# donydchen/matchnerf

Measured on AMD Instinct MI355X. Metric: rendered rays/sec (3-view, 64 samples/ray), higher is better.
Workload: dtype f32; 1 GPU

## Files before the change

matchnerf_amd/csrc/decoder.hip:

```cpp
#include "decoder_staged.hpp"

#define PP_STAGES 12
#define PP_PHASES 28
struct PPSched {
  int seg_first[PP_STAGES];
  int n_seg[PP_STAGES];
};

template <int SP>
struct SmemPP {
  static constexpr int TEAM = 128, TILE = 256;
  static constexpr int RING_FLOATS = 4 * SEG_CAP_FLOATS;
  static constexpr int TAIL_F = ((TAIL_FLOATS + 255) / 256) * 256;
  static constexpr int HDR_FLOATS = PP_STAGES * 256;
  static constexpr int RS_FLOATS = TILE * 4;
  static constexpr int TOTAL_FLOATS = RING_FLOATS + TAIL_F + HDR_FLOATS + RS_FLOATS + 64;
  static_assert(TEAM * 64 <= SEG_CAP_FLOATS, "a team's attention scratch must fit one ring slot");
  static_assert(TOTAL_FLOATS * 4 <= 160 * 1024, "LDS budget of one CU");
};
__device__ __host__ constexpr int pp_p0(int s, int fs = 2) {
  if (s == 0) return 1 + 8 * fs;
  constexpr int t[PP_STAGES] = {17, 33, 33, 33, 33, 33, 32, 33, 17, 33, 17, 9};
  return t[s];
}
__device__ __host__ constexpr int pp_stream_pieces(int k, int fs = 2) {
  if (k == 0) return 1 + 8 * fs;
  constexpr int t[20] = {17, 33, 33, 32, 33, 32, 33, 32, 33, 32, 33, 32, 32, 17, 33, 32, 17, 20, 9, 11};
  return t[k];
}
__device__ __host__ constexpr int pp_stream_off_floats(int k, int fs = 2) {
  int o = 0;
  for (int m = 0; m < k; ++m) o += pp_stream_pieces(m, fs) * 256;
  return o;
}
__device__ __host__ constexpr int pp_seg_first(int s) {
  constexpr int t[PP_STAGES] = {0, 1, 2, 4, 6, 8, 11, 10, 13, 14, 16, 18};
  return t[s];
}
__device__ __host__ constexpr int pp_seg_off_floats(int s, int i, int fs = 2) { return pp_stream_off_floats(pp_seg_first(s) + i, fs); }
constexpr int PP_DMA_IN_M = 0;
static_assert(PP_DMA_IN_M == 0, "requests inside matrix phases take single pieces 2 tw + half + 8 k");
__device__ __host__ constexpr int pp_km(int n) {
  const int enc_stage = 7;
  if (n < 3 || n > 11 || n == enc_stage + 1) return 0;
  const int fit = pp_p0(n) / 8;
  return fit < PP_DMA_IN_M ? fit : PP_DMA_IN_M;
}
__device__ __host__ constexpr int pp_p1(int s) {
  constexpr int t[PP_STAGES] = {0, 0, 32, 32, 32, 32, 32, 0, 0, 32, 20, 0};
  return t[s];
}


template <int CTRL, int ROW_MASK = 0xF>
__device__ __forceinline__ float dpp_get0(float v) {
  return __int_as_float(__builtin_amdgcn_update_dpp(0, __float_as_int(v), CTRL, ROW_MASK, 0xF, true));
}
__device__ __forceinline__ float readlane_f(float v, int l) {
  return __int_as_float(__builtin_amdgcn_readlane(__float_as_int(v), l));
}
__device__ __forceinline__ float wave_sum_dpp(float v) {
  v = dpp_group_sum<16>(v);
  return (readlane_f(v, 0) + readlane_f(v, 16)) + (readlane_f(v, 32) + readlane_f(v, 48));
}
__device__ __forceinline__ float wave_exclusive_sum_dpp(float v, int lane) {
  float x = dpp_get0<0x111>(v);
  const float c15 = readlane_f(v, 15), c31 = readlane_f(v, 31), c47 = readlane_f(v, 47);
  x = lane == 16 ? c15 : (lane == 32 ? c31 : (lane == 48 ? c47 : x));
  x += dpp_get0<0x111>(x);
  x += dpp_get0<0x112>(x);
  x += dpp_get0<0x114>(x);
  x += dpp_get0<0x118>(x);
  const float t0 = readlane_f(x, 15), t1 = readlane_f(x, 31), t2 = readlane_f(x, 47);
  const float t01 = t0 + t1;
  return x + (lane >= 48 ? t01 + t2 : (lane >= 32 ? t01 : (lane >= 16 ? t0 : 0.0f)));
}

template <int SP, bool PADDED>
__device__ __forceinline__ void ray_attention_pp(const float* q_lds, const float* k_lds, const float* vt_lds, float* o_lds,
                                                 int a_ray, int a_hp, int s_q, int lane, int S) {
  constexpr int G = SP / 4;
  constexpr int NH = SP >= 128 ? 1 : 2;
#pragma unroll 1
  for (int h0 = 0; h0 < 2; h0 += NH) {
    f32x4 sc[NH][G];
    float4 q4[NH];
    const float* kb[NH];
    const float* vb[NH];
#pragma unroll
    for (int hh = 0; hh < NH; ++hh) {
      const int head = 2 * a_hp + h0 + hh;
      q4[hh] = *reinterpret_cast<const float4*>(q_lds + s_q * 16 + head * 4);
      kb[hh] = k_lds + ((a_ray * 4 + head) * SP + (lane & 3)) * 4;
      vb[hh] = vt_lds + ((a_ray * 4 + head) * 4 + (lane & 3)) * SP;
    }
#pragma unroll
    for (int g = 0; g < G; g += 2) {
      float4 ka[NH], kc[NH];
      f32x4 ta[NH], tc[NH];
#pragma unroll
      for (int hh = 0; hh < NH; ++hh) {
        ka[hh] = *reinterpret_cast<const float4*>(kb[hh] + g * 16);
        kc[hh] = *reinterpret_cast<const float4*>(kb[hh] + g * 16 + 16);
      }
#pragma unroll
      for (int hh = 0; hh < NH; ++hh) {
        ta[hh] = mfma4(ka[hh].x, q4[hh].x, (f32x4){0.f, 0.f, 0.f, 0.f});
        tc[hh] = mfma4(kc[hh].x, q4[hh].x, (f32x4){0.f, 0.f, 0.f, 0.f});
      }
#pragma unroll
      for (int hh = 0; hh < NH; ++hh) {
        ta[hh] = mfma4(ka[hh].y, q4[hh].y, ta[hh]);
        tc[hh] = mfma4(kc[hh].y, q4[hh].y, tc[hh]);
      }
#pragma unroll
      for (int hh = 0; hh < NH; ++hh) {
        ta[hh] = mfma4(ka[hh].z, q4[hh].z, ta[hh]);
        tc[hh] = mfma4(kc[hh].z, q4[hh].z, tc[hh]);
      }
#pragma unroll
      for (int hh = 0; hh < NH; ++hh) {
        sc[hh][g] = mfma4(ka[hh].w, q4[hh].w, ta[hh]);
        sc[hh][g + 1] = mfma4(kc[hh].w, q4[hh].w, tc[hh]);
      }
    }
    float mx[NH];
#pragma unroll
    for (int hh = 0; hh < NH; ++hh) {
      float mx4[4] = {-3.0e38f, -3.0e38f, -3.0e38f, -3.0e38f};
      if constexpr (!PADDED) {
#pragma unroll
        for (int g = 0; g < G; ++g)
#pragma unroll
          for (int r = 0; r < 4; ++r) mx4[r] = fmaxf(mx4[r], sc[hh][g][r]);
      } else {
        int s_keys = S;
        asm volatile("" : "+s"(s_keys));
#pragma unroll
        for (int g = 0; g < G; ++g)
#pragma unroll
          for (int r = 0; r < 4; ++r) {
            const float v = (4 * g + r < s_keys) ? sc[hh][g][r] : -3.0e38f;
            sc[hh][g][r] = v;
            mx4[r] = fmaxf(mx4[r], v);
          }
      }
      mx[hh] = fmaxf(fmaxf(mx4[0], mx4[1]), fmaxf(mx4[2], mx4[3]));
    }
    float ls4[NH][4];
    f32x4 oa[NH], ob[NH];
#pragma unroll
    for (int hh = 0; hh < NH; ++hh) {
#pragma unroll
      for (int r = 0; r < 4; ++r) ls4[hh][r] = 0.f;
      oa[hh] = (f32x4){0.f, 0.f, 0.f, 0.f};
      ob[hh] = (f32x4){0.f, 0.f, 0.f, 0.f};
    }
#pragma unroll
    for (int g = 0; g < G; g += 2) {
      float4 va[NH], vc[NH];
#pragma unroll
      for (int hh = 0; hh < NH; ++hh) {
        va[hh] = *reinterpret_cast<const float4*>(vb[hh] + 4 * g);
        vc[hh] = *reinterpret_cast<const float4*>(vb[hh] + 4 * g + 4);
      }
#pragma unroll
      for (int u = 0; u < 2; ++u)
#pragma unroll
        for (int hh = 0; hh < NH; ++hh)
#pragma unroll
          for (int r = 0; r < 4; ++r) {
            const float pr = __builtin_amdgcn_exp2f(sc[hh][g + u][r] - mx[hh]);
            sc[hh][g + u][r] = pr;
            ls4[hh][r] += pr;
          }
#pragma unroll
      for (int hh = 0; hh < NH; ++hh) {
        oa[hh] = mfma4(va[hh].x, sc[hh][g][0], oa[hh]);
        ob[hh] = mfma4(vc[hh].x, sc[hh][g + 1][0], ob[hh]);
      }
#pragma unroll
      for (int hh = 0; hh < NH; ++hh) {
        oa[hh] = mfma4(va[hh].y, sc[hh][g][1], oa[hh]);
        ob[hh] = mfma4(vc[hh].y, sc[hh][g + 1][1], ob[hh]);
      }
#pragma unroll
      for (int hh = 0; hh < NH; ++hh) {
        oa[hh] = mfma4(va[hh].z, sc[hh][g][2], oa[hh]);
        ob[hh] = mfma4(vc[hh].z, sc[hh][g + 1][2], ob[hh]);
      }
#pragma unroll
      for (int hh = 0; hh < NH; ++hh) {
        oa[hh] = mfma4(va[hh].w, sc[hh][g][3], oa[hh]);
        ob[hh] = mfma4(vc[hh].w, sc[hh][g + 1][3], ob[hh]);
      }
    }
#pragma unroll
    for (int hh = 0; hh < NH; ++hh) {
      const int head = 2 * a_hp + h0 + hh;
      const float lsum = (ls4[hh][0] + ls4[hh][1]) + (ls4[hh][2] + ls4[hh][3]);
      const float il = 1.0f / lsum;
      *reinterpret_cast<float4*>(o_lds + s_q * 16 + head * 4) =
          make_float4((oa[hh][0] + ob[hh][0]) * il, (oa[hh][1] + ob[hh][1]) * il, (oa[hh][2] + ob[hh][2]) * il,
                      (oa[hh][3] + ob[hh][3]) * il);
    }
  }
}

template <bool PADDED, class Wait>
__device__ __forceinline__ void ray_attention_pp256(const float* q_lds, const float* k0, const float* vt0, const float* k1,
                                                    const float* vt1, float* o_lds, int a_hp, int s_q, int lane, int S, int first,
                                                    Wait wait_other) {
  constexpr int HS = 128, G = HS / 4;
  float m0 = -3.0e38f, m1 = -3.0e38f, l0 = 0.f, l1 = 0.f;
  f32x4 o0 = {0.f, 0.f, 0.f, 0.f}, o1 = {0.f, 0.f, 0.f, 0.f};
#pragma unroll 1
  for (int it = 0; it < 4; ++it) {
    if (it == 2) wait_other();
    const int half = it < 2 ? first : 1 - first;
    const int hsel = it & 1;
    const int head = 2 * a_hp + hsel;
    const float* kh = half == 0 ? k0 : k1;
    const float* vh = half == 0 ? vt0 : vt1;
    int n_keys = S - half * HS;
    n_keys = n_keys < 0 ? 0 : (n_keys > HS ? HS : n_keys);
    const float m_run = hsel ? m1 : m0, l_run = hsel ? l1 : l0;
    const float4 q4 = *reinterpret_cast<const float4*>(q_lds + s_q * 16 + head * 4);
    const float* kb = kh + (head * HS + (lane & 3)) * 4;
    const float* vb = vh + (head * 4 + (lane & 3)) * HS;
    f32x4 sc[G];
#pragma unroll
    for (int g = 0; g < G; g += 2) {
      const float4 ka = *reinterpret_cast<const float4*>(kb + g * 16);
      const float4 kc = *reinterpret_cast<const float4*>(kb + g * 16 + 16);
      f32x4 ta = mfma4(ka.x, q4.x, (f32x4){0.f, 0.f, 0.f, 0.f});
      f32x4 tc = mfma4(kc.x, q4.x, (f32x4){0.f, 0.f, 0.f, 0.f});
      ta = mfma4(ka.y, q4.y, ta);
      tc = mfma4(kc.y, q4.y, tc);
      ta = mfma4(ka.z, q4.z, ta);
      tc = mfma4(kc.z, q4.z, tc);
      sc[g] = mfma4(ka.w, q4.w, ta);
      sc[g + 1] = mfma4(kc.w, q4.w, tc);
    }
    float mx4[4] = {-3.0e38f, -3.0e38f, -3.0e38f, -3.0e38f};
    if constexpr (!PADDED) {
#pragma unroll
      for (int g = 0; g < G; ++g)
#pragma unroll
        for (int r = 0; r < 4; ++r) mx4[r] = fmaxf(mx4[r], sc[g][r]);
    } else {
      int s_keys = __builtin_amdgcn_readfirstlane(n_keys);
      asm volatile("" : "+s"(s_keys));
#pragma unroll
      for (int g = 0; g < G; ++g)
#pragma unroll
        for (int r = 0; r < 4; ++r) {
          const float v = (4 * g + r < s_keys) ? sc[g][r] : -3.0e38f;
          sc[g][r] = v;
          mx4[r] = fmaxf(mx4[r], v);
        }
    }
    const float m_new = fmaxf(m_run, fmaxf(fmaxf(mx4[0], mx4[1]), fmaxf(mx4[2], mx4[3])));
    float ls4[4] = {0.f, 0.f, 0.f, 0.f};
    f32x4 oa = {0.f, 0.f, 0.f, 0.f}, ob = {0.f, 0.f, 0.f, 0.f};
#pragma unroll
    for (int g = 0; g < G; g += 2) {
      const float4 va = *reinterpret_cast<const float4*>(vb + 4 * g);
      const float4 vc = *reinterpret_cast<const float4*>(vb + 4 * g + 4);
#pragma unroll
      for (int u = 0; u < 2; ++u)
#pragma unroll
        for (int r = 0; r < 4; ++r) {
          const float pr = __builtin_amdgcn_exp2f(sc[g + u][r] - m_new);
          sc[g + u][r] = pr;
          ls4[r] += pr;
        }
      oa = mfma4(va.x, sc[g][0], oa);
      ob = mfma4(vc.x, sc[g + 1][0], ob);
      oa = mfma4(va.y, sc[g][1], oa);
      ob = mfma4(vc.y, sc[g + 1][1], ob);
      oa = mfma4(va.z, sc[g][2], oa);
      ob = mfma4(vc.z, sc[g + 1][2], ob);
      oa = mfma4(va.w, sc[g][3], oa);
      ob = mfma4(vc.w, sc[g + 1][3], ob);
    }
    const float f_old = __builtin_amdgcn_exp2f(m_run - m_new);
    const float l_new = l_run * f_old + ((ls4[0] + ls4[1]) + (ls4[2] + ls4[3]));
    f32x4 o_new;
#pragma unroll
    for (int d = 0; d < 4; ++d) o_new[d] = (hsel ? o1[d] : o0[d]) * f_old + (oa[d] + ob[d]);
    if (hsel) {
      m1 = m_new, l1 = l_new, o1 = o_new;
    } else {
      m0 = m_new, l0 = l_new, o0 = o_new;
    }
  }
  {
    const float i0 = 1.0f / l0, i1 = 1.0f / l1;
    *reinterpret_cast<float4*>(o_lds + s_q * 16 + (2 * a_hp) * 4) = make_float4(o0[0] * i0, o0[1] * i0, o0[2] * i0, o0[3] * i0);
    *reinterpret_cast<float4*>(o_lds + s_q * 16 + (2 * a_hp + 1) * 4) = make_float4(o1[0] * i1, o1[1] * i1, o1[2] * i1, o1[3] * i1);
  }
}

template <int SP, int FS = 2, bool POSES = false, int NPK = 3>
__global__ __launch_bounds__(512, 2) void decoder_pp_kernel(
    mnerf_decoder D, DecSched sch, PPSched pps, mnerf_view view0, mnerf_rays Rl, const float* __restrict__ cond,
    float* __restrict__ out_rgb, float* __restrict__ out_depth, float* __restrict__ out_opacity,
    float* __restrict__ dbg_rgb_s, float* __restrict__ dbg_sigma, const float* __restrict__ ext_ndc,
    const float* __restrict__ ext_dir) {
  constexpr int Sp = SP;
  using SM = SmemPP<SP>;
  constexpr int TEAM = SM::TEAM;
  extern __shared__ __attribute__((aligned(16))) float smem[];
  const unsigned ring_lds = __builtin_amdgcn_groupstaticsize();
  const unsigned tail_lds = ring_lds + SM::RING_FLOATS * 4u;
  const unsigned hdr_lds = tail_lds + SM::TAIL_F * 4u;
  float* tail = smem + SM::RING_FLOATS;
  float* rs_all = tail + SM::TAIL_F + SM::HDR_FLOATS;
  float* ln_lds = rs_all + SM::RS_FLOATS;

  const int tid = threadIdx.x;
  const int lane0 = tid & 63;
  const int wave = __builtin_amdgcn_readfirstlane(tid >> 6);
  const int team = wave >> 2, tw = wave & 3;
  const mnerf_rays& R = Rl;
  const int S = R.n_samples;
  constexpr bool WIDE = SP == 256;
  static_assert(!WIDE || (!POSES && FS == 2), "the 256-sample instance exists for the shipped shape without a pose table");
  const int rays_per_team = WIDE ? 0 : TEAM / Sp, rays_per_tile = WIDE ? 1 : 2 * rays_per_team;
  const int n_tiles = (R.n_rays + rays_per_tile - 1) / rays_per_tile;
  const int CS = D.cond_stride;
  const float freq_mul = R.legacy_coord ? 1.0f : 3.14159265358979323846f;
  const float wm1 = (float)(R.width - 1), hm1 = (float)(R.height - 1);
  float* rs_lds = rs_all + team * TEAM * 4;
  float* att = smem + (team == 0 ? 3 : 2) * SEG_CAP_FLOATS;
  float* k_lds = att;
  float* vt_lds = att + TEAM * 16;
  float* q_lds = att + TEAM * 32;
  float* o_lds = att + TEAM * 48;
  const float* k_other = smem + (team == 0 ? 2 : 3) * SEG_CAP_FLOATS;
  const float* vt_other = k_other + TEAM * 16;
  float* rows_lds = smem + 1 * SEG_CAP_FLOATS + team * 4096;
  const unsigned rows_lds_addr = ring_lds + (unsigned)(1 * SEG_CAP_FLOATS + team * 4096) * 4u;

#define PP_SLOT_LDS(s_, i_) (ring_lds + (unsigned)(2 * ((s_)&1) + (i_)) * (SEG_CAP_FLOATS * 4u))
#define PP_HDR_LDS(s_) (hdr_lds + (unsigned)(s_) * 1024u)
#define PP_SEG_SRC(s_, i_) (D.wstream + pp_seg_off_floats(s_, i_, FS))

  if (tid < SMALL_FIXED) ln_lds[tid] = D.small_[tid];
  if (tid < 2) reinterpret_cast<unsigned*>(ln_lds)[48 + tid] = 0u;
  const unsigned team_ctr_lds = hdr_lds + (unsigned)(SM::HDR_FLOATS + SM::RS_FLOATS + 48 + team) * 4u;
  int team_epoch = 0;
  const unsigned other_ctr_lds = hdr_lds + (unsigned)(SM::HDR_FLOATS + SM::RS_FLOATS + 48 + (1 - team)) * 4u;
  int tile_it = 0;
  auto wait_other_team = [&](int arrivals) {
    const int want = 4 * arrivals;
    for (;;) {
      unsigned v;
      asm volatile("ds_read_b32 %0, %1\n\ts_waitcnt lgkmcnt(0)" : "=v"(v) : "v"(other_ctr_lds) : "memory");
      if ((int)((unsigned)__builtin_amdgcn_readfirstlane((int)v) - (unsigned)want) >= 0) break;
      __builtin_amdgcn_s_sleep(1);
    }
  };
  {
    const unsigned voff = (unsigned)lane0 * 16u;
    for (int p = wave; p < pp_stream_pieces(19); p += 8)
      glds16_s(D.wstream + pp_stream_off_floats(19, FS) + p * 256, voff, __builtin_amdgcn_readfirstlane(tail_lds + (unsigned)p * 1024u));
    for (int s = wave; s < PP_STAGES; s += 8) glds16_s(PP_SEG_SRC(s, 0), voff, __builtin_amdgcn_readfirstlane(PP_HDR_LDS(s)));
    for (int p = wave; p < pp_p0(0, FS); p += 8)
      glds16_s(PP_SEG_SRC(0, 0) + p * 256, voff, __builtin_amdgcn_readfirstlane(PP_SLOT_LDS(0, 0) + (unsigned)p * 1024u));
  }
  segment_wait();
  __syncthreads();
  if (team == 1) __syncthreads();

  int tile_begin = blockIdx.x, tile_end = n_tiles, tile_step = gridDim.x;
  if (gridDim.x >= 8) {
    const int xcd = blockIdx.x & 7;
    tile_begin = (int)((long long)n_tiles * xcd / 8) + (int)(blockIdx.x >> 3);
    tile_end = (int)((long long)n_tiles * (xcd + 1) / 8);
    tile_step = ((int)gridDim.x - xcd + 7) >> 3;
  }
#ifdef MNERF_TIMELINE
  int pp_tl_tile = -1, pp_ph = 0;
#define PP_STAMPED(sync_)                                                                                      \
  do {                                                                                                         \
    unsigned long long* o_ = (sch.tl && lane0 == 0 && blockIdx.x < 32 && pp_tl_tile >= 0 && pp_tl_tile < 4)     \
                                 ? sch.tl + ((((size_t)blockIdx.x * 4 + pp_tl_tile) * 8 + wave) * PP_PHASES + pp_ph) * 2 \
                                 : nullptr;                                                                    \
    __builtin_amdgcn_sched_barrier(0);                                                                         \
    if (o_) o_[0] = __builtin_amdgcn_s_memtime();                                                              \
    sync_;                                                                                                     \
    if (o_) o_[1] = __builtin_amdgcn_s_memtime();                                                              \
    __builtin_amdgcn_sched_barrier(0);                                                                         \
    ++pp_ph;                                                                                                   \
  } while (0)
#else
#define PP_STAMPED(sync_)                    \
  do {                                       \
    __builtin_amdgcn_sched_barrier(0);       \
    sync_;                                   \
    __builtin_amdgcn_sched_barrier(0);       \
  } while (0)
#endif
#define PP_SYNC() PP_STAMPED(__syncthreads())
#define PP_TSYNC() PP_STAMPED(wave_group_sync(team_ctr_lds, 4, team_epoch, (int)hw_lane()))
#define PP_NOSYNC() PP_STAMPED((void)0)
  auto stage_dma = [&](int s, int half) {
    const unsigned voff = hw_lane() * 16u;
    int twl = tw;
    asm volatile("" : "+s"(twl));
    for (int i = 0; i < 2; ++i) {
      const int pieces = i == 0 ? pp_p0(s, FS) : pp_p1(s);
      const unsigned base = PP_SLOT_LDS(s, i);
      const int first = half == 2 ? twl : 2 * twl + half, step = half == 2 ? 4 : 8;
      const int n_runs = pieces >> 2;
      for (int r = first; r <= n_runs; r += step) {
        const unsigned off = (unsigned)r * 4096u;
        if (r < n_runs)
          glds16_sv4(D.wstream, voff, (unsigned)pp_seg_off_floats(s, i, FS) * 4u + off, __builtin_amdgcn_readfirstlane(base + off));
        else
          for (int p = 4 * n_runs; p < pieces; ++p)
            glds16_sv(D.wstream, voff, (unsigned)pp_seg_off_floats(s, i, FS) * 4u + (unsigned)p * 1024u,
                      __builtin_amdgcn_readfirstlane(base + (unsigned)p * 1024u));
      }
    }
  };
  int dma_k = 0;
  auto stage_piece = [&](int s, int half, int k) {
    const int i = k / 5;
    const int pcs = i == 0 ? pp_p0(s, FS) : pp_p1(s);
    int twl = tw;
    asm volatile("" : "+s"(twl));
    const int pce = 2 * twl + half + 8 * (k % 5);
    if (pcs > 0 && pce < pcs) {
      const unsigned vo = hw_lane() * 16u;
      glds16_s(PP_SEG_SRC(s, i) + pce * 256, vo, __builtin_amdgcn_readfirstlane(PP_SLOT_LDS(s, i) + (unsigned)pce * 1024u));
    }
  };
  auto dma_some = [&](int sa, int sb, int n) {
#pragma unroll
    for (int q = 0; q < n; ++q) {
      if (dma_k >= 10) break;
      __builtin_amdgcn_sched_barrier(0);
      if (team == 0) {
        if (sa >= 0) stage_piece(sa, 1, dma_k);
      } else {
        if (sb >= 0) stage_piece(sb, 0, dma_k);
      }
      __builtin_amdgcn_sched_barrier(0);
      ++dma_k;
    }
  };
#define PP_SEGMENT_WAIT() segment_wait()
  auto burst_from = [&](int s, int half, int k0) {
    if (k0 == 0) {
      stage_dma(s, half);
      return;
    }
#pragma unroll
    for (int k = k0; k < 10; ++k) stage_piece(s, half, k);
  };
  auto stage_piece_m = [&](int s, int k, unsigned lane_addr, unsigned lane_addr_base) {
    int twl = tw;
    asm volatile("" : "+s"(twl));
    const int pce = 2 * twl + (1 - team) + 8 * k;
    glds16_s(reinterpret_cast<const float*>(reinterpret_cast<const char*>(PP_SEG_SRC(s, 0) + pce * 256) - lane_addr_base), lane_addr,
             __builtin_amdgcn_readfirstlane(PP_SLOT_LDS(s, 0) + (unsigned)pce * 1024u));
  };
  auto pp_m_dma = [&](int s, int n_units, int i, unsigned lane_addr, unsigned lane_addr_base) {
#pragma unroll
    for (int j = 0; j < pp_km(s + 1); ++j)
      if ((j * (n_units / 2)) / pp_km(s + 1) == i) stage_piece_m(s + 1, j, lane_addr, lane_addr_base);
  };
#define PP_BEGIN_V(stage_)                                                          \
  do {                                                                              \
    if (team == 0) burst_from(stage_, 1, pp_km(stage_));                            \
    else if ((stage_) + 1 < PP_STAGES) burst_from((stage_) + 1, 0, pp_km((stage_) + 1)); \
  } while (0)
  (void)dma_some;
#define PP_DMA(sa_, sb_, n_) do {} while (0)
#define PP_END_V(sa_, next_stage_)                                  \
  do {                                                              \
    if (team == 1) { if ((next_stage_) >= 0 && (sa_) < 0) stage_dma(next_stage_, 0); } \
    else PP_SEGMENT_WAIT();                                         \
    PP_SYNC();                                                      \
  } while (0)
#define PP_END_M()                   \
  do {                               \
    if (team == 1) PP_SEGMENT_WAIT();   \
    PP_SYNC();                       \
  } while (0)
#define PP_PRIO_UP() do {} while (0)
#define PP_PRIO_DOWN() do {} while (0)
#define PP_MFMA_(NMB_, NS0_, NS1_, acc_, base0_, base1_, hs_) ksteps_presplit2<NMB_, NS0_, NS1_, NPK>(acc_, base0_, base1_, lane, hs_)
#define PP_MFMA_HOOKED(NMB_, NS0_, NS1_, acc_, s_, hdr_bytes_, hs_)                                                      \
  ksteps_presplit2<NMB_, NS0_, NS1_, NPK>(acc_, PP_SLOT_LDS(s_, 0) + (hdr_bytes_), PP_SLOT_LDS(s_, 1), lane, hs_,        \
                                     [&](int i_, unsigned la_, unsigned lb_) { pp_m_dma(s_, ((NS0_) + (NS1_)) * (NMB_), i_, la_, lb_); })
#define PP_MFMA(NMB_, NS0_, NS1_, acc_, s_, hdr_bytes_, hs_)                                                   \
  do {                                                                                                         \
    PP_PRIO_UP();                                                                                              \
    PP_MFMA_HOOKED(NMB_, NS0_, NS1_, acc_, s_, hdr_bytes_, hs_);                                                \
    PP_PRIO_DOWN();                                                                                            \
  } while (0)
#define PP_MFMA1(NS0_, acc_, s_, hdr_bytes_, hs_)                                                              \
  do {                                                                                                         \
    PP_PRIO_UP();                                                                                              \
    PP_MFMA_HOOKED(1, NS0_, 0, acc_, s_, hdr_bytes_, hs_);                                                      \
    PP_PRIO_DOWN();                                                                                            \
  } while (0)

  bool rows_in_lds = false;
  for (int tile = tile_begin; tile < tile_end; tile += tile_step) {
#ifdef MNERF_TIMELINE
    ++pp_tl_tile;
    pp_ph = 0;
#endif
    const bool has_next = tile + tile_step < tile_end;
    int tile_pose = 0;
    if constexpr (POSES)
      tile_pose = pose_of_ray(Rl, (tile * rays_per_tile + team * rays_per_team < Rl.n_rays) ? tile * rays_per_tile + team * rays_per_team : Rl.n_rays - 1);
#define PP_TILE_RAYS(NAME_)                                  \
  mnerf_rays NAME_ = Rl;                                     \
  if constexpr (POSES) rays_for_pose(NAME_, Rl, tile_pose)
    const int lane = (int)hw_lane();
    const int n = lane & 31, hl = lane >> 5;
    const unsigned voff = (unsigned)lane * 16u;
    const int s_local = tw * 32 + n;
    const int ray_t = WIDE ? 0 : s_local / Sp;
    const int jp = WIDE ? team * TEAM + s_local : s_local - ray_t * Sp;
    const int ray_raw = tile * rays_per_tile + team * rays_per_team + ray_t;
    const bool ray_ok = ray_raw < R.n_rays;
    const int ray = ray_ok ? ray_raw : (R.n_rays - 1);
    const int j = jp < S ? jp : (S - 1);
    const size_t gs = (size_t)ray * S + j;

    float4 cpre[2 * FS];
    float n_valid;
    {
      const float* crow = (FS == 2 && rows_in_lds) ? rows_lds + s_local * CS : cond + gs * CS;
#pragma unroll
      for (int i = 0; i < 2 * FS; ++i) {
        const int o = 16 * (i >> 1) + 8 * hl + 4 * (i & 1);
        cpre[i] = (o + 4 <= CS) ? *reinterpret_cast<const float4*>(crow + o) : make_float4(0.f, 0.f, 0.f, 0.f);
      }
      const float* mrow = crow + (D.cond_dim - D.n_views);
      float nv = 0.0f;
      for (int v = 0; v < D.n_views; ++v) nv += mrow[v];
      n_valid = nv;
    }
    float x, y, z, enc_max;
    const bool q_valid = n_valid > 1.0f;

    dma_k = 0;
    PartsH hs[8];
    f32x16 film[4];
    int ecf;
    {
#pragma unroll
      for (int t = 0; t < FS; ++t) {
        const float vt[8] = {cpre[2 * t].x, cpre[2 * t].y, cpre[2 * t].z, cpre[2 * t].w,
                             cpre[2 * t + 1].x, cpre[2 * t + 1].y, cpre[2 * t + 1].z, cpre[2 * t + 1].w};
        hs[t] = split8h(vt, (float)(1 << (H16_TARGET_EXP - 1)));
      }
      const int ew = header_ew(PP_HDR_LDS(0));
      ecf = -(ew + (H16_TARGET_EXP - 1));
      bias_init_h<4>(film, PP_HDR_LDS(0), hl, pow2i(ew + (H16_TARGET_EXP - 1)));
    }
    PP_END_V(-1, 1);
    PP_MFMA(4, FS, 0, film, 0, 1024u, hs);
    __builtin_amdgcn_sched_barrier(0);
    if (ext_ndc) {
      x = ext_ndc[gs * 3 + 0];
      y = ext_ndc[gs * 3 + 1];
      z = ext_ndc[gs * 3 + 2];
    } else {
      PP_TILE_RAYS(Rt);
      const RayGeom g = make_ray(Rt, ray);
      const float dpt = sample_depth(Rt, ray, j);
      float wx_, wy_, wz_;
      ray_point(g, dpt, wx_, wy_, wz_);
      project(view0, wx_, wy_, wz_, wm1, hm1, x, y, z);
    }
    enc_max = fmaxf(fmaxf(1.0f, fabsf(x)), fmaxf(fabsf(y), fabsf(z)));
    __builtin_amdgcn_sched_barrier(0);
    PP_END_M();
    PP_BEGIN_V(1);
    f32x16 acc[4];
    int ew_cur = 0, ec, em;
    auto split_enc_half = [&](int half, float mult) {
      float xo = x, yo = y, zo = z;
      asm volatile("" : "+v"(xo), "+v"(yo), "+v"(zo));
      const EncBase encb = enc_base(xo, yo, zo, freq_mul);
      const f32x16 e = half == 0 ? enc_block16_L10<0>(encb, hl, xo, yo, zo) : enc_block16_L10<16>(encb, hl, xo, yo, zo);
      float v[8];
#pragma unroll
      for (int r = 0; r < 8; ++r) v[r] = e[r];
      hs[2 * half] = split8h(v, mult);
#pragma unroll
      for (int r = 0; r < 8; ++r) v[r] = e[8 + r];
      hs[2 * half + 1] = split8h(v, mult);
    };
#define PP_ENC_MFMA(acc_, s_, mult_)                                                                             \
  do {                                                                                                           \
    PP_PRIO_UP();                                                                                                \
    PP_MFMA_(4, 2, 0, acc_, PP_SLOT_LDS(s_, 0) + 1024u, PP_SLOT_LDS(s_, 1), hs);                                 \
    PP_PRIO_DOWN();                                                                                              \
    __builtin_amdgcn_sched_barrier(0);                                                                           \
    split_enc_half(1, mult_);                                                                                    \
    __builtin_amdgcn_sched_barrier(0);                                                                           \
    PP_PRIO_UP();                                                                                                \
    PP_MFMA_(4, 2, 0, acc_, PP_SLOT_LDS(s_, 0) + 1024u + 8 * H16_UNIT_BYTES, PP_SLOT_LDS(s_, 1), hs + 2);         \
    PP_PRIO_DOWN();                                                                                              \
  } while (0)
    auto split_blocks = [&](const f32x16 (&b)[4], float mult, int sa, int sb) {
      PP_DMA(sa, sb, 3);
#pragma unroll
      for (int m = 0; m < 4; ++m) {
        float v[8];
#pragma unroll
        for (int r = 0; r < 8; ++r) v[r] = b[m][r];
        hs[2 * m] = split8h(v, mult);
        PP_DMA(sa, sb, 1);
#pragma unroll
        for (int r = 0; r < 8; ++r) v[r] = b[m][8 + r];
        hs[2 * m + 1] = split8h(v, mult);
        PP_DMA(sa, sb, 1);
      }
    };
    auto film_relu = [&](f32x16 (&dst)[4]) -> float {
      float mx = 0.0f;
#pragma unroll
      for (int m = 0; m < 4; ++m)
#pragma unroll
        for (int r = 0; r < 16; ++r) {
          const float t = fmaxf(acc[m][r] * film[m][r], 0.0f);
          dst[m][r] = t;
          mx = fmaxf(mx, t);
        }
      return pair_max(mx);
    };
    em = gain_exp(enc_max);
    const float mult_l0 = pow2i(em);
    PP_DMA(1, 2, 4);
    split_enc_half(0, mult_l0);
    PP_DMA(1, 2, 4);
    ew_cur = header_ew(PP_HDR_LDS(1));
    bias_init_h<4>(acc, PP_HDR_LDS(1), hl, pow2i(ew_cur + em));
    ec = -em - ew_cur + ecf;
    PP_END_V(1, 2);
    PP_ENC_MFMA(acc, 1, mult_l0);
    PP_END_M();
    float hmax;
#define PP_HIDDEN_LAYER(ST_)                                                \
  do {                                                                      \
    PP_BEGIN_V(ST_);                                                        \
    hmax = film_relu(acc);                                                  \
    em = gain_exp(hmax);                                                    \
    split_blocks(acc, pow2i(em), ST_, (ST_) + 1);                           \
    ew_cur = header_ew(PP_HDR_LDS(ST_));                                    \
    bias_init_h<4>(acc, PP_HDR_LDS(ST_), hl, pow2i(ew_cur + (em - ec)));    \
    ec = ec - em - ew_cur + ecf;                                            \
    PP_END_V(ST_, (ST_) + 1);                                               \
    PP_MFMA(4, 4, 4, acc, ST_, 1024u, hs);            \
    PP_END_M();                                                             \
  } while (0)
    PP_HIDDEN_LAYER(2);
    PP_HIDDEN_LAYER(3);
    PP_HIDDEN_LAYER(4);
    PP_HIDDEN_LAYER(5);
#undef PP_HIDDEN_LAYER
    int eg;
    PP_BEGIN_V(6);
    {
      hmax = film_relu(acc);
      eg = gain_exp(fmaxf(enc_max, hmax * pow2i(ec)));
      split_blocks(acc, pow2i(eg + ec), 6, 7);
      ew_cur = header_ew(PP_HDR_LDS(7));
      bias_init_h<4>(acc, PP_HDR_LDS(7), hl, pow2i(ew_cur + eg));
    }
    PP_END_V(6, 7);
    PP_MFMA(4, 4, 4, acc, 6, 0u, hs);
    PP_END_M();
    PP_BEGIN_V(7);
    const float mult_l5 = pow2i(eg);
    PP_DMA(7, 8, 4);
    split_enc_half(0, mult_l5);
    ec = -eg - ew_cur + ecf;
    PP_END_V(7, 8);
    PP_ENC_MFMA(acc, 7, mult_l5);
    PP_END_M();
    PP_BEGIN_V(8);
    hmax = film_relu(acc);
    const int em5 = gain_exp(hmax);
    split_blocks(acc, pow2i(em5), 8, 9);
    f32x16 al[1];
    const int ew_a = header_ew(PP_HDR_LDS(8));
    bias_init_h<1>(al, PP_HDR_LDS(8), hl, pow2i(ew_a + em5 - ec));
    PP_END_V(8, 9);
    PP_MFMA1(8, al, 8, 1024u, hs);
    PP_END_M();
    float av[8];
    PP_BEGIN_V(9);
    {
      const float ca = pow2i(ec - em5 - ew_a);
#pragma unroll
      for (int r = 0; r < 8; ++r) {
        float t = al[0][r] * ca;
        t = D.raytrans_elu ? (t > 0.0f ? t : (expf(t) - 1.0f)) : fmaxf(t, 0.0f);
        av[r] = t;
      }
      if (D.raytrans_posenc) {
        const float* tab = D.small_ + SMALL_FIXED + (size_t)j * 16;
#pragma unroll
        for (int r = 0; r < 8; ++r) av[r] += tab[(r & 3) + 8 * (r >> 2) + 4 * hl];
      }
      ew_cur = header_ew(PP_HDR_LDS(9));
      bias_init_h<4>(acc, PP_HDR_LDS(9), hl, pow2i(ew_cur + (em5 - ec)));
    }
    const int ecfeat = ec - em5 - ew_cur;
    PP_END_V(9, 10);
    PP_MFMA(4, 4, 4, acc, 9, 1024u, hs);
    PP_END_M();
    int egv, ecv;
    PartsH hsd;
    f32x16 hv[2];
    PP_BEGIN_V(10);
    {
      float dx, dy, dz;
      if (ext_ndc) {
        dx = ext_dir[gs * 3 + 0];
        dy = ext_dir[gs * 3 + 1];
        dz = ext_dir[gs * 3 + 2];
      } else {
        PP_TILE_RAYS(Rt);
        const RayGeom g = make_ray(Rt, ray);
        const float rn = fmaxf(sqrtf(g.rx * g.rx + g.ry * g.ry + g.rz * g.rz), 1e-12f);
        const float ux = g.rx / rn, uy = g.ry / rn, uz = g.rz / rn;
        dx = ux * view0.extr[0] + uy * view0.extr[1] + uz * view0.extr[2];
        dy = ux * view0.extr[4] + uy * view0.extr[5] + uz * view0.extr[6];
        dz = ux * view0.extr[8] + uy * view0.extr[9] + uz * view0.extr[10];
      }
      egv = gain_exp(fmaxf(1.0f, sample_absmax<4>(acc) * pow2i(ecfeat)));
      split_blocks(acc, pow2i(egv + ecfeat), 10, 11);
      const float v[8] = {hl ? 0.0f : dx, hl ? 0.0f : dy, hl ? 0.0f : dz, 0.0f, 0.0f, 0.0f, 0.0f, 0.0f};
      hsd = split8h(v, pow2i(egv));
      const int ew = header_ew(PP_HDR_LDS(10));
      bias_init_h<2>(hv, PP_HDR_LDS(10), hl, pow2i(ew + egv));
      ecv = -egv - ew;
    }
    PP_END_V(10, 11);
    PP_MFMA(2, 4, 4, hv, 10, 1024u, hs);
    ksteps_presplit<2, 1>(hv, PP_SLOT_LDS(10, 1) + 8 * H16_UNIT_BYTES, lane, &hsd);
    PP_END_M();
    f32x16 c3[1];
    float cc;
    PP_BEGIN_V(11);
    {
#pragma unroll
      for (int m = 0; m < 2; ++m)
#pragma unroll
        for (int r = 0; r < 16; ++r) hv[m][r] = fmaxf(hv[m][r], 0.0f);
      const int emr = gain_exp(sample_absmax<2>(hv));
      const float mult = pow2i(emr);
#pragma unroll
      for (int m = 0; m < 2; ++m) {
        float v[8];
#pragma unroll
        for (int r = 0; r < 8; ++r) v[r] = hv[m][r];
        hs[2 * m] = split8h(v, mult);
#pragma unroll
        for (int r = 0; r < 8; ++r) v[r] = hv[m][8 + r];
        hs[2 * m + 1] = split8h(v, mult);
      }
      const int ew = header_ew(PP_HDR_LDS(11));
      bias_init_h<1>(c3, PP_HDR_LDS(11), hl, pow2i(ew + emr - ecv));
      cc = pow2i(ecv - emr - ew);
    }
    PP_END_V(11, -1);
    {
      PP_MFMA1(4, c3, 11, 1024u, hs);
      if (hl == 0) {
        const float cr = 1.0f / (1.0f + expf(-c3[0][0] * cc));
        const float cg = 1.0f / (1.0f + expf(-c3[0][1] * cc));
        const float cb = 1.0f / (1.0f + expf(-c3[0][2] * cc));
        rs_lds[s_local * 4 + 0] = cr;
        rs_lds[s_local * 4 + 1] = cg;
        rs_lds[s_local * 4 + 2] = cb;
        if (dbg_rgb_s && ray_ok && jp < S) {
          dbg_rgb_s[gs * 3 + 0] = cr;
          dbg_rgb_s[gs * 3 + 1] = cg;
          dbg_rgb_s[gs * 3 + 2] = cb;
        }
      }
    }
    if (team == 1) {
      segment_wait();
      PP_TSYNC();
    } else {
      PP_SYNC();
    }
    bool next_rows = false;
    if (FS == 2 && S == Sp && has_next) {
      const int first_ray = (tile + tile_step) * rays_per_tile + team * rays_per_team;
      next_rows = WIDE ? first_ray < R.n_rays : first_ray + rays_per_team <= R.n_rays;
      if (next_rows) {
        const float* src = cond + ((size_t)first_ray * S + (WIDE ? team * TEAM : 0)) * CS;
        const int pieces = (TEAM * CS) >> 8;
        for (int p = tw; p < pieces; p += 4) glds16_s_stream(src + p * 256, voff, __builtin_amdgcn_readfirstlane(rows_lds_addr + (unsigned)p * 1024u));
      }
    }
    f32x16 qkv[2];
    qkv[0] = (f32x16)(0.0f);
    qkv[1] = (f32x16)(0.0f);
#pragma unroll
    for (int r = 0; r < 8; ++r) step2(qkv, tail + TAIL_QKV, r, lane, av[r]);
    const float qs = q_valid ? 0.5f * 1.4426950408889634f : 0.0f;
#pragma unroll
    for (int hh = 0; hh < 2; ++hh) {
      const int head = hl + 2 * hh;
      constexpr int SPT = WIDE ? TEAM : SP;
      const int jt = WIDE ? s_local : jp;
      *reinterpret_cast<float4*>(k_lds + ((ray_t * 4 + head) * SPT + jt) * 4) =
          make_float4(qkv[0][8 + 4 * hh], qkv[0][9 + 4 * hh], qkv[0][10 + 4 * hh], qkv[0][11 + 4 * hh]);
      float* vcol = vt_lds + (ray_t * 4 + head) * 4 * SPT + jt;
      vcol[0] = qkv[1][4 * hh];
      vcol[SPT] = qkv[1][4 * hh + 1];
      vcol[2 * SPT] = qkv[1][4 * hh + 2];
      vcol[3 * SPT] = qkv[1][4 * hh + 3];
      *reinterpret_cast<float4*>(q_lds + s_local * 16 + head * 4) =
          make_float4(qkv[0][4 * hh] * qs, qkv[0][4 * hh + 1] * qs, qkv[0][4 * hh + 2] * qs, qkv[0][4 * hh + 3] * qs);
    }
    PP_TSYNC();
    {
      int a_ray, a_hp, a_jq;
      if constexpr (SP >= 64) {
        constexpr int CH = (WIDE ? TEAM : SP) / 64;
        int idx = tw;
        const int chunk = idx % CH;
        idx /= CH;
        a_hp = idx & 1;
        a_ray = idx >> 1;
        a_jq = chunk * 64 + lane;
      } else {
        a_ray = tw;
        a_hp = lane >> 5;
        a_jq = lane & 31;
      }
      if constexpr (WIDE) {
        const float* k0 = team == 0 ? k_lds : k_other;
        const float* vt0 = team == 0 ? vt_lds : vt_other;
        const float* k1 = team == 0 ? k_other : k_lds;
        const float* vt1 = team == 0 ? vt_other : vt_lds;
        const int other_t1 = team == 0 ? 4 * tile_it + 2 : 3 * tile_it + 1;
        auto wait = [&]() { wait_other_team(other_t1); };
        if (S == Sp)
          ray_attention_pp256<false>(q_lds, k0, vt0, k1, vt1, o_lds, a_hp, a_jq, lane, S, team, wait);
        else
          ray_attention_pp256<true>(q_lds, k0, vt0, k1, vt1, o_lds, a_hp, a_jq, lane, S, team, wait);
      } else {
        if (S == Sp)
          ray_attention_pp<SP, false>(q_lds, k_lds, vt_lds, o_lds, a_ray, a_hp, a_ray * Sp + a_jq, lane, S);
        else
          ray_attention_pp<SP, true>(q_lds, k_lds, vt_lds, o_lds, a_ray, a_hp, a_ray * Sp + a_jq, lane, S);
      }
    }
    segment_wait();
    PP_TSYNC();
    {
      float ofc[8];
      {
        const float4* src = reinterpret_cast<const float4*>(o_lds + s_local * 16 + 8 * hl);
        const float4 t0 = src[0], t1 = src[1];
        ofc[0] = t0.x; ofc[1] = t0.y; ofc[2] = t0.z; ofc[3] = t0.w;
        ofc[4] = t1.x; ofc[5] = t1.y; ofc[6] = t1.z; ofc[7] = t1.w;
      }
      float yv[8];
      {
        f32x16 t1 = (f32x16)(0.0f);
#pragma unroll
        for (int t = 0; t < 8; ++t) step1(t1, tail + TAIL_FCO, t, lane, ofc[t]);
        float xs = 0.f;
#pragma unroll
        for (int r = 0; r < 8; ++r) {
          yv[r] = t1[r] + av[r];
          xs += yv[r];
        }
        xs = pair_sum(xs);
        const float mean = xs * (1.0f / 16.0f);
        float var = 0.f;
#pragma unroll
        for (int r = 0; r < 8; ++r) {
          const float dlt = yv[r] - mean;
          var += dlt * dlt;
        }
        var = pair_sum(var);
        const float rstd = 1.0f / sqrtf(var * (1.0f / 16.0f) + 1e-6f);
#pragma unroll
        for (int r = 0; r < 8; ++r) {
          const int o = (r & 3) + 8 * (r >> 2) + 4 * hl;
          yv[r] = (yv[r] - mean) * rstd * ln_lds[o] + ln_lds[16 + o];
        }
      }
      float sigma;
      {
        f32x16 t2 = (f32x16)(0.0f);
#pragma unroll
        for (int r = 0; r < 8; ++r) step1(t2, tail + TAIL_OA0, r, lane, yv[r]);
        step1(t2, tail + TAIL_OA0, 8, lane, hl ? 0.0f : 1.0f);
        f32x16 t3 = (f32x16)(0.0f);
#pragma unroll
        for (int r = 0; r < 8; ++r) {
          float t = t2[r];
          t = D.raytrans_elu ? (t > 0.0f ? t : (expf(t) - 1.0f)) : fmaxf(t, 0.0f);
          step1(t3, tail + TAIL_OA2, r, lane, t);
        }
        step1(t3, tail + TAIL_OA2, 8, lane, hl ? 0.0f : 1.0f);
        sigma = fmaxf(t3[0], 0.0f);
      }
      if (D.density_maskfill && n_valid < 1.0f) sigma = 0.0f;
      if (hl == 0) {
        rs_lds[s_local * 4 + 3] = sigma;
        if (dbg_sigma && ray_ok && jp < S) dbg_sigma[gs] = sigma;
      }
    }
    if (team == 1 && has_next) stage_dma(0, 2);
    PP_TSYNC();
    PP_TILE_RAYS(Rt);
    const int t4_rays = WIDE ? ((team == 1 && tw == 0) ? 1 : 0) : rays_per_team;
    const float* rs_ray = WIDE ? rs_all : rs_lds;
    if (WIDE && t4_rays) wait_other_team(3 * tile_it + 3);
    for (int rt = WIDE ? 0 : tw; rt < t4_rays; rt += 4) {
      const int rr = tile * rays_per_tile + team * rays_per_team + rt;
      if (rr >= R.n_rays || !out_rgb) continue;
      float rlen = 1.0f;
      if (!D.wo_render_interval) {
        const RayGeom gg = make_ray(Rt, rr);
        rlen = sqrtf(gg.rx * gg.rx + gg.ry * gg.ry + gg.rz * gg.rz);
      }
      float carry = 0.f, ar = 0.f, ag = 0.f, ab = 0.f, ad = 0.f, ao = 0.f;
      for (int j0 = 0; j0 < S; j0 += 64) {
        const int jj = j0 + lane;
        const bool ok = jj < S;
        float4 c = make_float4(0.f, 0.f, 0.f, 0.f);
        float dd = 0.f;
        if (ok) {
          c = reinterpret_cast<const float4*>(rs_ray)[rt * Sp + jj];
          dd = sample_depth(Rt, rr, jj);
          if (!D.wo_render_interval) {
            const float intv = (jj + 1 < S) ? (sample_depth(Rt, rr, jj + 1) - dd) : 1e10f;
            c.w = c.w * (intv * rlen);
          }
        }
        const float excl = carry + wave_exclusive_sum_dpp(c.w, lane);
        const float w = ok ? expf(-excl) * (1.0f - expf(-c.w)) : 0.0f;
        ar += w * c.x;
        ag += w * c.y;
        ab += w * c.z;
        ad += w * dd;
        ao += w;
        carry = readlane_f(excl + c.w, 63);
      }
      ar = wave_sum_dpp(ar);
      ag = wave_sum_dpp(ag);
      ab = wave_sum_dpp(ab);
      ad = wave_sum_dpp(ad);
      ao = wave_sum_dpp(ao);
      if (lane == 0) {
        const float bg = D.setbg_opaque ? (1.0f - ao) : 0.0f;
        out_rgb[(size_t)rr * 3 + 0] = ar + bg;
        out_rgb[(size_t)rr * 3 + 1] = ag + bg;
        out_rgb[(size_t)rr * 3 + 2] = ab + bg;
        out_depth[rr] = ad;
        out_opacity[rr] = ao;
      }
    }
    rows_in_lds = next_rows;
    ++tile_it;
    if (team == 1) {
      segment_wait();
      PP_SYNC();
    } else {
      PP_NOSYNC();
    }
  }
  if (team == 0) __syncthreads();
#undef PP_END_V
#undef PP_DMA
#undef PP_BEGIN_V
#undef PP_END_M
#undef PP_SYNC
#undef PP_TSYNC
#undef PP_NOSYNC
#undef PP_STAMPED
#undef PP_ENC_MFMA
#undef PP_MFMA_
#undef PP_PRIO_UP
#undef PP_PRIO_DOWN
#undef PP_MFMA
#undef PP_MFMA1
#undef PP_HDR_LDS
#undef PP_TILE_RAYS
#undef PP_SEG_SRC
#undef PP_SLOT_LDS
}

extern "C" int64_t mnerf_decoder_wstream_floats(int32_t cond_dim, int32_t cond_stride, int32_t L_3D,
                                                int32_t wstream_format) {
  if (!known_format(wstream_format)) return -1;
  if (L_3D < 0 || L_3D > 16 || cond_dim < 1 || cond_stride < cond_dim) return -1;
  mnerf_decoder d = {};
  d.cond_dim = cond_dim;
  d.cond_stride = cond_stride;
  d.L_3D = L_3D;
  d.wstream_format = wstream_format;
  DecSched s;
  return build_schedule(&d, &s);
}

static int pp_film_steps(const mnerf_decoder* dec, const DecSched& sch, int Sp) {
  const int pp_max_s = mnerf_tune().decoder_pp_max_s < 256 ? mnerf_tune().decoder_pp_max_s : 256;
  const int fs = sch.film_steps;
  const bool f16 = dec->wstream_format == MNERF_WSTREAM_F16X2 || dec->wstream_format == MNERF_WSTREAM_F16X1;
  const bool ok = f16 && Sp > 0 && Sp <= pp_max_s && dec->L_3D == 10 &&
                  (fs == 2 || ((fs == 3 || fs == 4) && Sp == 64)) && dec->cond_stride <= 16 * fs && sch.enc_steps == 4 &&
                  sch.n_seg == 20 && mnerf_tune().decoder_pp;
  return ok ? fs : 0;
}

template <int SP, int FS, bool POSES, int NPK>
static void launch_pp_instance(const DecCall& c, const DecSched& sch, const PPSched& pps) {
  const int rpt = 256 / SP;
  const int tiles = (c.rays->n_rays + rpt - 1) / rpt;
  const int cus = mnerf_tune().decoder_pp_grid > 0 ? mnerf_tune().decoder_pp_grid : 1;
  const int grid = tiles < cus ? tiles : cus;
  const size_t lds = SmemPP<SP>::TOTAL_FLOATS * sizeof(float);
  static std::atomic<unsigned long long> attr_set{0};
  if (mnerf_once_per_device(attr_set))
    (void)hipFuncSetAttribute((const void*)decoder_pp_kernel<SP, FS, POSES, NPK>, hipFuncAttributeMaxDynamicSharedMemorySize, (int)lds);
  hipLaunchKernelGGL((decoder_pp_kernel<SP, FS, POSES, NPK>), dim3(grid), dim3(512), lds, (hipStream_t)c.stream, *c.dec, sch, pps, *c.view0,
                     *c.rays, c.cond, c.rgb, c.depth, c.opacity, c.rgb_s, c.sigma, c.ext_ndc, c.ext_dir);
}

static int launch_pp(const DecCall& c, const DecSched& sch, int Sp, int fs) {
  const char* who = c.who;
  const mnerf_decoder* dec = c.dec;
  PPSched pps;
  const int first[PP_STAGES] = {0, 1, 2, 4, 6, 8, 11, 10, 13, 14, 16, 18};
  const int nseg[PP_STAGES] = {1, 1, 2, 2, 2, 2, 2, 1, 1, 2, 2, 1};
  for (int i = 0; i < PP_STAGES; ++i) {
    pps.seg_first[i] = first[i], pps.n_seg[i] = nseg[i];
    MNERF_REQUIRE((sch.seg_floats[first[i]] >> 8) == pp_p0(i, fs) && (nseg[i] == 2 ? (sch.seg_floats[first[i] + 1] >> 8) : 0) == pp_p1(i),
                  MNERF_E_RANGE, "%s: weight schedule does not match the ping-pong kernel (stage %d)", who, i);
    MNERF_REQUIRE(first[i] == pp_seg_first(i), MNERF_E_RANGE, "%s: stage table of the ping-pong kernel (stage %d)", who, i);
  }
  for (int k = 0; k < 20; ++k)
    MNERF_REQUIRE(sch.seg_off[k] == pp_stream_off_floats(k, fs) && (sch.seg_floats[k] >> 8) == pp_stream_pieces(k, fs), MNERF_E_RANGE,
                  "%s: weight stream layout does not match the ping-pong kernel (segment %d)", who, k);
  if (dec->wstream_format == MNERF_WSTREAM_F16X1) {
    MNERF_REQUIRE(fs == 2 && !c.rays->pose_table && Sp <= 128, MNERF_E_UNSUPPORTED,
                  "%s: the one-product fp16 mode (MNERF_WSTREAM_F16X1) is built for <= 5 source views, sample_intvs <= 128, without a "
                  "pose table", who);
    if (Sp == 32)
      launch_pp_instance<32, 2, false, 1>(c, sch, pps);
    else if (Sp == 64)
      launch_pp_instance<64, 2, false, 1>(c, sch, pps);
    else
      launch_pp_instance<128, 2, false, 1>(c, sch, pps);
  } else if (c.rays->pose_table) {
    MNERF_REQUIRE(fs == 2 && (Sp == 32 || Sp == 64 || Sp == 128), MNERF_E_UNSUPPORTED,
                  "%s: pose tables are built for <= 5 source views and sample_intvs <= 128", who);
    if (Sp == 32)
      launch_pp_instance<32, 2, true, 3>(c, sch, pps);
    else if (Sp == 64)
      launch_pp_instance<64, 2, true, 3>(c, sch, pps);
    else
      launch_pp_instance<128, 2, true, 3>(c, sch, pps);
  } else if (fs == 3)
    launch_pp_instance<64, 3, false, 3>(c, sch, pps);
  else if (fs == 4)
    launch_pp_instance<64, 4, false, 3>(c, sch, pps);
  else if (Sp == 32)
    launch_pp_instance<32, 2, false, 3>(c, sch, pps);
  else if (Sp == 64)
    launch_pp_instance<64, 2, false, 3>(c, sch, pps);
  else if (Sp == 128)
    launch_pp_instance<128, 2, false, 3>(c, sch, pps);
  else
    launch_pp_instance<256, 2, false, 3>(c, sch, pps);
  return mnerf_check_launch(who);
}

static int launch_decoder(const DecCall& c) {
  int Sp;
  DecSched sch;
  if (const int err = check_decoder_call(c, &Sp, &sch)) return err;
  if (c.rays->n_rays == 0) return MNERF_OK;
  if (const int fs = pp_film_steps(c.dec, sch, Sp)) return launch_pp(c, sch, Sp, fs);
  return launch_staged<0>(c, sch, Sp);
}

bool mnerf_decoder_takes_pose_table(const mnerf_decoder* dec, int n_samples) {
  if (!known_format(dec->wstream_format) || dec->wstream_format == MNERF_WSTREAM_F16X1 || dec->L_3D < 0 || dec->L_3D > 16) return false;
  DecSched sch;
  if (build_schedule(dec, &sch) <= 0) return false;
  const int Sp = pick_padded_samples(n_samples);
  return (Sp == 32 || Sp == 64 || Sp == 128) && pp_film_steps(dec, sch, Sp) == 2;
}

extern "C" int mnerf_decoder_chunk(const mnerf_decoder* dec, const mnerf_view* view0,
                                   const mnerf_rays* rays, const float* cond, float* rgb,
                                   float* depth, float* opacity, float* dbg_rgb_s,
                                   float* dbg_sigma, void* stream) {
  MNERF_REQUIRE(dec && view0 && rays, MNERF_E_NULL, "mnerf_decoder_chunk: NULL argument struct");
  MNERF_REQUIRE(rgb && depth && opacity && cond, MNERF_E_NULL, "mnerf_decoder_chunk: NULL buffer");
  MNERF_REQUIRE(rays->legacy_coord == 0 || rays->n_samples >= 2, MNERF_E_RANGE,
                "mnerf_decoder_chunk: legacy depth sampling needs S >= 2");
  return launch_decoder({"mnerf_decoder_chunk", dec, view0, rays, cond, rgb, depth, opacity, dbg_rgb_s, dbg_sigma,
                         nullptr, nullptr, nullptr, stream});
}

extern "C" int mnerf_decoder_samples(const mnerf_decoder* dec, int32_t n_rays, int32_t n_samples,
                                     int32_t legacy_coord, const float* x_ndc, const float* dir,
                                     const float* cond, float* rgb_s, float* sigma, void* stream) {
  MNERF_REQUIRE(dec, MNERF_E_NULL, "mnerf_decoder_samples: dec is NULL");
  MNERF_REQUIRE(n_rays >= 0 && n_samples >= 1, MNERF_E_RANGE, "mnerf_decoder_samples: n_rays=%d S=%d", n_rays, n_samples);
  if (n_rays == 0) return MNERF_OK;
  MNERF_REQUIRE(x_ndc && dir && rgb_s && sigma, MNERF_E_NULL, "mnerf_decoder_samples: NULL buffer");
  mnerf_rays rays = {};
  rays.n_rays = n_rays;
  rays.n_samples = n_samples;
  rays.height = rays.width = 2;
  rays.legacy_coord = legacy_coord ? 1 : 0;
  const mnerf_view none = {};
  MNERF_REQUIRE(cond, MNERF_E_NULL, "mnerf_decoder_samples: cond is NULL");
  return launch_decoder({"mnerf_decoder_samples", dec, &none, &rays, cond, nullptr, nullptr, nullptr, rgb_s, sigma,
                         x_ndc, dir, nullptr, stream});
}
```

Measured before the change: 13.26 million rays/s.

## Defer ray compositing into next tile's MFMA phases and move DMA issue to team 0

```diff
diff --git a/matchnerf_amd/csrc/decoder.hip b/matchnerf_amd/csrc/decoder.hip
--- a/matchnerf_amd/csrc/decoder.hip
+++ b/matchnerf_amd/csrc/decoder.hip
@@ -327,6 +327,7 @@
   const int S = R.n_samples;
   constexpr bool WIDE = SP == 256;
   static_assert(!WIDE || (!POSES && FS == 2), "the 256-sample instance exists for the shipped shape without a pose table");
+  constexpr bool DEFER = !WIDE;
   const int rays_per_team = WIDE ? 0 : TEAM / Sp, rays_per_tile = WIDE ? 1 : 2 * rays_per_team;
   const int n_tiles = (R.n_rays + rays_per_tile - 1) / rays_per_tile;
   const int CS = D.cond_stride;
@@ -341,7 +342,6 @@
   const float* k_other = smem + (team == 0 ? 2 : 3) * SEG_CAP_FLOATS;
   const float* vt_other = k_other + TEAM * 16;
   float* rows_lds = smem + 1 * SEG_CAP_FLOATS + team * 4096;
-  const unsigned rows_lds_addr = ring_lds + (unsigned)(1 * SEG_CAP_FLOATS + team * 4096) * 4u;
 
 #define PP_SLOT_LDS(s_, i_) (ring_lds + (unsigned)(2 * ((s_)&1) + (i_)) * (SEG_CAP_FLOATS * 4u))
 #define PP_HDR_LDS(s_) (hdr_lds + (unsigned)(s_) * 1024u)
@@ -510,6 +510,67 @@
     PP_PRIO_DOWN();                                                                                            \
   } while (0)
 
+  auto pose_of_tile = [&](int t) -> int {
+    if constexpr (POSES)
+      return pose_of_ray(Rl, (t * rays_per_tile + team * rays_per_team < Rl.n_rays) ? t * rays_per_tile + team * rays_per_team : Rl.n_rays - 1);
+    else
+      return 0;
+  };
+#define PP_TILE_RAYS_OF(NAME_, POSE_)                        \
+  mnerf_rays NAME_ = Rl;                                     \
+  if constexpr (POSES) rays_for_pose(NAME_, Rl, POSE_)
+  auto composite_tile = [&](int ct, int cpose) {
+    const int lane = (int)hw_lane();
+    PP_TILE_RAYS_OF(Rt, cpose);
+    const int t4_rays = WIDE ? ((team == 1 && tw == 0) ? 1 : 0) : rays_per_team;
+    const float* rs_ray = WIDE ? rs_all : rs_lds;
+    if (WIDE && t4_rays) wait_other_team(3 * tile_it + 3);
+    for (int rt = WIDE ? 0 : tw; rt < t4_rays; rt += 4) {
+      const int rr = ct * rays_per_tile + team * rays_per_team + rt;
+      if (rr >= R.n_rays || !out_rgb) continue;
+      float rlen = 1.0f;
+      if (!D.wo_render_interval) {
+        const RayGeom gg = make_ray(Rt, rr);
+        rlen = sqrtf(gg.rx * gg.rx + gg.ry * gg.ry + gg.rz * gg.rz);
+      }
+      float carry = 0.f, ar = 0.f, ag = 0.f, ab = 0.f, ad = 0.f, ao = 0.f;
+      for (int j0 = 0; j0 < S; j0 += 64) {
+        const int jj = j0 + lane;
+        const bool ok = jj < S;
+        float4 c = make_float4(0.f, 0.f, 0.f, 0.f);
+        float dd = 0.f;
+        if (ok) {
+          c = reinterpret_cast<const float4*>(rs_ray)[rt * Sp + jj];
+          dd = sample_depth(Rt, rr, jj);
+          if (!D.wo_render_interval) {
+            const float intv = (jj + 1 < S) ? (sample_depth(Rt, rr, jj + 1) - dd) : 1e10f;
+            c.w = c.w * (intv * rlen);
+          }
+        }
+        const float excl = carry + wave_exclusive_sum_dpp(c.w, lane);
+        const float w = ok ? expf(-excl) * (1.0f - expf(-c.w)) : 0.0f;
+        ar += w * c.x;
+        ag += w * c.y;
+        ab += w * c.z;
+        ad += w * dd;
+        ao += w;
+        carry = readlane_f(excl + c.w, 63);
+      }
+      ar = wave_sum_dpp(ar);
+      ag = wave_sum_dpp(ag);
+      ab = wave_sum_dpp(ab);
+      ad = wave_sum_dpp(ad);
+      ao = wave_sum_dpp(ao);
+      if (lane == 0) {
+        const float bg = D.setbg_opaque ? (1.0f - ao) : 0.0f;
+        out_rgb[(size_t)rr * 3 + 0] = ar + bg;
+        out_rgb[(size_t)rr * 3 + 1] = ag + bg;
+        out_rgb[(size_t)rr * 3 + 2] = ab + bg;
+        out_depth[rr] = ad;
+        out_opacity[rr] = ao;
+      }
+    }
+  };
   bool rows_in_lds = false;
   for (int tile = tile_begin; tile < tile_end; tile += tile_step) {
 #ifdef MNERF_TIMELINE
@@ -517,12 +578,13 @@
     pp_ph = 0;
 #endif
     const bool has_next = tile + tile_step < tile_end;
-    int tile_pose = 0;
-    if constexpr (POSES)
-      tile_pose = pose_of_ray(Rl, (tile * rays_per_tile + team * rays_per_team < Rl.n_rays) ? tile * rays_per_tile + team * rays_per_team : Rl.n_rays - 1);
-#define PP_TILE_RAYS(NAME_)                                  \
-  mnerf_rays NAME_ = Rl;                                     \
-  if constexpr (POSES) rays_for_pose(NAME_, Rl, tile_pose)
+    const bool has_prev = DEFER && tile != tile_begin;
+#define PP_DEFERRED_T4(TEAM_)                                                                                  \
+  do {                                                                                                         \
+    if (team == (TEAM_) && has_prev) composite_tile(tile - tile_step, pose_of_tile(tile - tile_step));         \
+  } while (0)
+    const int tile_pose = pose_of_tile(tile);
+#define PP_TILE_RAYS(NAME_) PP_TILE_RAYS_OF(NAME_, tile_pose)
     const int lane = (int)hw_lane();
     const int n = lane & 31, hl = lane >> 5;
     const unsigned voff = (unsigned)lane * 16u;
@@ -567,6 +629,7 @@
       ecf = -(ew + (H16_TARGET_EXP - 1));
       bias_init_h<4>(film, PP_HDR_LDS(0), hl, pow2i(ew + (H16_TARGET_EXP - 1)));
     }
+    PP_DEFERRED_T4(0);
     PP_END_V(-1, 1);
     PP_MFMA(4, FS, 0, film, 0, 1024u, hs);
     __builtin_amdgcn_sched_barrier(0);
@@ -702,6 +765,7 @@
     PP_END_M();
     float av[8];
     PP_BEGIN_V(9);
+    PP_DEFERRED_T4(1);
     {
       const float ca = pow2i(ec - em5 - ew_a);
 #pragma unroll
@@ -802,12 +866,16 @@
     }
     bool next_rows = false;
     if (FS == 2 && S == Sp && has_next) {
-      const int first_ray = (tile + tile_step) * rays_per_tile + team * rays_per_team;
-      next_rows = WIDE ? first_ray < R.n_rays : first_ray + rays_per_team <= R.n_rays;
-      if (next_rows) {
-        const float* src = cond + ((size_t)first_ray * S + (WIDE ? team * TEAM : 0)) * CS;
-        const int pieces = (TEAM * CS) >> 8;
-        for (int p = tw; p < pieces; p += 4) glds16_s_stream(src + p * 256, voff, __builtin_amdgcn_readfirstlane(rows_lds_addr + (unsigned)p * 1024u));
+      for (int t = team; t < 2; ++t) {
+        const int first_ray = (tile + tile_step) * rays_per_tile + t * rays_per_team;
+        const bool rows_t = WIDE ? first_ray < R.n_rays : first_ray + rays_per_team <= R.n_rays;
+        if (t == team) next_rows = rows_t;
+        if (rows_t && team == 0) {
+          const float* src = cond + ((size_t)first_ray * S + (WIDE ? t * TEAM : 0)) * CS;
+          const int pieces = (TEAM * CS) >> 8;
+          const unsigned dst = ring_lds + (unsigned)(1 * SEG_CAP_FLOATS + t * 4096) * 4u;
+          for (int p = tw; p < pieces; p += 4) glds16_s_stream(src + p * 256, voff, __builtin_amdgcn_readfirstlane(dst + (unsigned)p * 1024u));
+        }
       }
     }
     f32x16 qkv[2];
@@ -865,7 +933,7 @@
           ray_attention_pp<SP, true>(q_lds, k_lds, vt_lds, o_lds, a_ray, a_hp, a_ray * Sp + a_jq, lane, S);
       }
     }
-    segment_wait();
+    if (team == 0) segment_wait();
     PP_TSYNC();
     {
       float ofc[8];
@@ -924,61 +992,12 @@
         if (dbg_sigma && ray_ok && jp < S) dbg_sigma[gs] = sigma;
       }
     }
-    if (team == 1 && has_next) stage_dma(0, 2);
+    if (team == 0 && has_next) stage_dma(0, 2);
     PP_TSYNC();
-    PP_TILE_RAYS(Rt);
-    const int t4_rays = WIDE ? ((team == 1 && tw == 0) ? 1 : 0) : rays_per_team;
-    const float* rs_ray = WIDE ? rs_all : rs_lds;
-    if (WIDE && t4_rays) wait_other_team(3 * tile_it + 3);
-    for (int rt = WIDE ? 0 : tw; rt < t4_rays; rt += 4) {
-      const int rr = tile * rays_per_tile + team * rays_per_team + rt;
-      if (rr >= R.n_rays || !out_rgb) continue;
-      float rlen = 1.0f;
-      if (!D.wo_render_interval) {
-        const RayGeom gg = make_ray(Rt, rr);
-        rlen = sqrtf(gg.rx * gg.rx + gg.ry * gg.ry + gg.rz * gg.rz);
-      }
-      float carry = 0.f, ar = 0.f, ag = 0.f, ab = 0.f, ad = 0.f, ao = 0.f;
-      for (int j0 = 0; j0 < S; j0 += 64) {
-        const int jj = j0 + lane;
-        const bool ok = jj < S;
-        float4 c = make_float4(0.f, 0.f, 0.f, 0.f);
-        float dd = 0.f;
-        if (ok) {
-          c = reinterpret_cast<const float4*>(rs_ray)[rt * Sp + jj];
-          dd = sample_depth(Rt, rr, jj);
-          if (!D.wo_render_interval) {
-            const float intv = (jj + 1 < S) ? (sample_depth(Rt, rr, jj + 1) - dd) : 1e10f;
-            c.w = c.w * (intv * rlen);
-          }
-        }
-        const float excl = carry + wave_exclusive_sum_dpp(c.w, lane);
-        const float w = ok ? expf(-excl) * (1.0f - expf(-c.w)) : 0.0f;
-        ar += w * c.x;
-        ag += w * c.y;
-        ab += w * c.z;
-        ad += w * dd;
-        ao += w;
-        carry = readlane_f(excl + c.w, 63);
-      }
-      ar = wave_sum_dpp(ar);
-      ag = wave_sum_dpp(ag);
-      ab = wave_sum_dpp(ab);
-      ad = wave_sum_dpp(ad);
-      ao = wave_sum_dpp(ao);
-      if (lane == 0) {
-        const float bg = D.setbg_opaque ? (1.0f - ao) : 0.0f;
-        out_rgb[(size_t)rr * 3 + 0] = ar + bg;
-        out_rgb[(size_t)rr * 3 + 1] = ag + bg;
-        out_rgb[(size_t)rr * 3 + 2] = ab + bg;
-        out_depth[rr] = ad;
-        out_opacity[rr] = ao;
-      }
-    }
+    if (!DEFER || !has_next) composite_tile(tile, tile_pose);
     rows_in_lds = next_rows;
     ++tile_it;
     if (team == 1) {
-      segment_wait();
       PP_SYNC();
     } else {
       PP_NOSYNC();
@@ -1001,6 +1020,8 @@
 #undef PP_MFMA1
 #undef PP_HDR_LDS
 #undef PP_TILE_RAYS
+#undef PP_TILE_RAYS_OF
+#undef PP_DEFERRED_T4
 #undef PP_SEG_SRC
 #undef PP_SLOT_LDS
 }
```

Result: no change. 13.24 million rays/s, median of 4 (-0.1%).
